# learningmatter-mit/surface-sampling

Hardware: AMD Instinct MI355X
Metric: MC energy-evaluations/sec (SrTiO3(001) ~250-atom slabs, 3-model PaiNN ensemble E+F incl. neighbor list) (higher is better)
Workload: dtype f32 via fp16x2-split MFMA (3 products), fp32 accumulate; neighbor decisions f64; 1 GPU; SrTiO3(001) PaiNN x3, 256 batched independent chains per GPU (BASELINE configs[3]), 248-272 atoms/chain; chains_per_gpu=256, atoms_per_gpu=66503, edges_per_gpu=2747786, slots_per_gpu=2836316, models=3, streams_per_gpu=2, parallelism=one GPU, no collective

## Files before the change

### surface-sampling_amd/csrc/api_batch.hip

```cpp
#include <cmath>
#include <cstdio>

#include "cell_dev.h"
#include "ewald_dev.h"

using namespace vssr;

extern "C" {

int vssr_batch_upload(vssr_handle *h, int32_t n_cfg, const int32_t *n_atoms, const int32_t *Z, const double *pos,
                      const double *cell, const uint8_t *pbc) {
    if (int rc = check_kind(h, KINDS_EVAL, __func__)) return rc;
    if (n_cfg < 1 || !n_atoms || !Z || !pos || !cell || !pbc) return set_err(h, VSSR_E_BADARG, "null or empty batch");
    VSSR_HIP(h, hipSetDevice(h->device));
    VSSR_HIP(h, hipStreamSynchronize(h->stream));
    h->batch_valid = false;
    h->ran = false;
    h->md_vel_valid = false;
    std::vector<int> start(n_cfg + 1, 0);
    for (int b = 0; b < n_cfg; ++b) {
        if (n_atoms[b] < 1) return set_err(h, VSSR_E_BADARG, "configuration %d has %d atoms", b, n_atoms[b]);
        if ((int64_t)start[b] + n_atoms[b] > 2000000000LL) return set_err(h, VSSR_E_BADARG, "batch too large");
        start[b + 1] = start[b] + n_atoms[b];
    }
// ... 573 lines not shown
        if (l == 0 && h->l0_used)
            return set_err(h, VSSR_E_STATE, "phi0 is not materialised (layer-0 species factorisation is active)");
        src = sv.phi[l]; per_atom = F3;
    }
    else if ((l = layer_of("s_msg")) >= 0) { src = sv.s_msg[l]; per_atom = F; }
    else if ((l = layer_of("v_msg")) >= 0) { src = sv.v_msg[l]; per_atom = F3; }
    else if ((l = layer_of("s_upd")) >= 0) { src = sv.s_in[l + 1]; per_atom = F; }
    else if ((l = layer_of("v_upd")) >= 0) {
        if (l == h->num_conv - 1 && !h->debug_keep)
            return set_err(h, VSSR_E_STATE, "v_upd of the last block is not materialised (nothing consumes it; create the handle with VSSR_DEBUG_KEEP=1)");
        src = sv.v_in[l + 1]; per_atom = F3;
    }
    else if (nm == "e_atom") { src = sv.e_atom; per_atom = 1; }
    else if (nm == "sbar_msg0") { src = sv.sbar_msg_l0; per_atom = F; }
    else if (nm == "vbar_msg0") { src = sv.vbar_msg; per_atom = F3; }
    else return set_err(h, VSSR_E_BADARG, "unknown intermediate '%s'", name);
    size_t n = N * per_atom;
    *n_out = (int64_t)n;
    if (!dst) return VSSR_OK;
    if ((int64_t)n > cap) return set_err(h, VSSR_E_BADARG, "buffer too small for '%s'", name);
    VSSR_HIP(h, hipMemcpy(dst, src + (size_t)model * n, n * sizeof(float), hipMemcpyDeviceToHost));
    return VSSR_OK;
}

}
```

### surface-sampling_amd/csrc/api_painn.hip

```cpp
#include <cmath>

#include "vssr_internal.h"

namespace vssr {

static void transpose(const float *src, int rows, int cols, float *dst) {
    for (int r = 0; r < rows; ++r)
        for (int c = 0; c < cols; ++c) dst[(size_t)c * rows + r] = src[(size_t)r * cols + c];
}

static int upload_weights(vssr_handle *h, const vssr_painn_config *cfg) {
    const int M = cfg->n_models, L = cfg->num_conv, R = cfg->n_rbf, H = cfg->readout_hidden, NE = cfg->n_embed;
    const size_t per_layer = (size_t)F * F + F + (size_t)F3 * F + F3 + (size_t)F3 * R + F3 + 2 * (size_t)F * F +
                             (size_t)F * 2 * F + F + (size_t)F3 * F + F3;
    const size_t blob_len = (size_t)NE * F + L * per_layer + (size_t)H * F + H + H + 1;
    if (cfg->weights_len != blob_len)
        return set_err(h, VSSR_E_BADARG, "weights_len %llu does not match the layout (%zu floats)",
                       (unsigned long long)cfg->weights_len, blob_len);
    const size_t t_per_layer = (size_t)F * F + (size_t)F * F3 + 2 * (size_t)F * F + (size_t)2 * F * F + (size_t)F * F3;
    const size_t img_len = blob_len + L * t_per_layer + (size_t)F * H;
    std::vector<float> img(img_len * M);
    std::vector<ModelW> table(M);
    if (h->weights.ensure(img.size() * sizeof(float)))
        return set_err(h, VSSR_E_NOMEM, "weights: out of device memory");
// ... 123 lines not shown
}

static void read_env_knobs(vssr_handle *h) {
    if (const char *e = getenv("VSSR_PAINN_PATH")) h->painn_general = h->painn_general || strcmp(e, "general") == 0;
    if (const char *e = getenv("VSSR_EDGE_IMPL")) h->edge_impl = (strcmp(e, "gather") == 0) ? 0 : 1;
    if (const char *e = getenv("VSSR_L0_FACTORISE")) h->l0_enabled = atoi(e);
    if (h->painn_general) h->l0_enabled = 0;
    if (const char *e = getenv("VSSR_UPD_SAVE")) h->upd_save = atoi(e);
    if (const char *e = getenv("VSSR_DEBUG_KEEP")) h->debug_keep = atoi(e);
    if (const char *e = getenv("VSSR_EDGE_FS16_MAX")) h->fs16_max_atoms = atoi(e);
    if (const char *e = getenv("VSSR_EDGE_FS8_MAX")) h->fs8_max_atoms = atoi(e);
    if (const char *e = getenv("VSSR_EDGE_BWD_MPASS")) h->bwd_multi_pass = atoi(e);
    if (const char *e = getenv("VSSR_EDGE_SUB_CHUNK")) { const int c = atoi(e); if (c >= 8) { h->sub_chunk_fwd = c; h->sub_chunk_bwd = c; } }
    if (const char *e = getenv("VSSR_EDGE_FWD_2PASS")) { const int w = atoi(e); h->fwd_two_pass = (w == 8 || w == 16) ? w : w ? 16 : 0; }
    if (const char *e = getenv("VSSR_EDGE_FWD_GRID")) h->edge_fwd_grid = max(atoi(e), 0);
}

}

using namespace vssr;

extern "C" {

int vssr_create(const vssr_painn_config *cfg, vssr_handle **out) {
    if (!cfg || !out) return set_err(nullptr, VSSR_E_BADARG, "null argument");
    *out = nullptr;
    if (cfg->struct_size != sizeof(vssr_painn_config))
        return set_err(nullptr, VSSR_E_BADARG, "vssr_painn_config size mismatch (%u vs %zu)", cfg->struct_size,
                       sizeof(vssr_painn_config));
    if (cfg->feat_dim < 16 || cfg->feat_dim > 256 || cfg->feat_dim % 16 != 0 || cfg->n_rbf < 1 || cfg->n_rbf > 32)
// ... 39 lines not shown
```

### surface-sampling_amd/csrc/mfma16.h

```cpp
#ifndef VSSR_MFMA16_H
#define VSSR_MFMA16_H
#include "vssr_internal.h"

namespace vssr {

typedef float f32x4 __attribute__((ext_vector_type(4)));
typedef float f32x2 __attribute__((ext_vector_type(2)));
typedef unsigned u32x4 __attribute__((ext_vector_type(4)));
typedef unsigned u32x2 __attribute__((ext_vector_type(2)));
typedef _Float16 f16x8 __attribute__((ext_vector_type(8)));
typedef _Float16 f16x2 __attribute__((ext_vector_type(2)));

constexpr int TA = 32;
constexpr int NW = 8;
constexpr int NTHREADS = 64 * NW;
constexpr int PADH = 8;

#ifndef VSSR_FAST_SIGMOID
#define VSSR_FAST_SIGMOID 1
#endif
__device__ __forceinline__ float sigm(float x) {
#if VSSR_FAST_SIGMOID && defined(__HIP_DEVICE_COMPILE__)
    constexpr float C_HI = -1.44269502162933349609375f;
    constexpr float C_LO = -1.9259629911266175e-08f;
// ... 120 lines not shown
    }
}
template <int NROWS, class Sat>
__device__ __forceinline__ void rows_store_split(const Planes &P, int col0, const float4 (&v)[NROWS * (F / 4) / NTHREADS],
                                                 Sat &sat) {
    constexpr int NIT = NROWS * (F / 4) / NTHREADS;
#pragma unroll
    for (int it = 0; it < NIT; ++it) {
        const int idx = threadIdx.x + it * NTHREADS;
        store_split4<SAT_COOP>(P, idx >> 5, col0 + 4 * (idx & 31), v[it], sat);
    }
}

constexpr int FT = F + 4;
template <int NROWS, class Fn>
__device__ __forceinline__ void stage_rows(const float *T, Fn fn) {
    constexpr int NIT = NROWS * (F / 4) / NTHREADS;
    static_assert(NROWS * (F / 4) % NTHREADS == 0, "tile pass must divide evenly");
#pragma unroll
    for (int it = 0; it < NIT; ++it) {
        const int idx = threadIdx.x + it * NTHREADS, row = idx >> 5, c4 = idx & 31;
        fn(row, 4 * c4, *reinterpret_cast<const float4 *>(T + row * FT + 4 * c4));
    }
}

template <int NROWS, class Ld, class St>
__device__ __forceinline__ void stage_rows_residual(const float *T, Ld ld, St st) {
    constexpr int NIT = NROWS * (F / 4) / NTHREADS;
    static_assert(NROWS * (F / 4) % NTHREADS == 0, "tile pass must divide evenly");
    float4 r[NIT];
#pragma unroll
    for (int it = 0; it < NIT; ++it) {
        const int idx = threadIdx.x + it * NTHREADS;
        r[it] = ld(idx >> 5, 4 * (idx & 31));
    }
#pragma unroll
    for (int it = 0; it < NIT; ++it) {
        const int idx = threadIdx.x + it * NTHREADS, row = idx >> 5, c4 = idx & 31;
        st(row, 4 * c4, *reinterpret_cast<const float4 *>(T + row * FT + 4 * c4), r[it]);
// ... 38 lines not shown
```

### surface-sampling_amd/csrc/painn.hip

```cpp
#include "vssr_internal.h"

namespace vssr {

constexpr int T = NODE_TILE;
constexpr int RB = 21;
constexpr int ECHUNK = 16;
constexpr float PI_F = 3.14159265358979323846f;

__device__ inline float sigmoidf_(float x) { return 1.f / (1.f + expf(-x)); }
__device__ inline float swishf_(float x) { return x * sigmoidf_(x); }
__device__ inline float dswishf_(float x) {
    float sg = sigmoidf_(x);
    return sg * fmaf(x, 1.f - sg, 1.f);
}

__global__ void __launch_bounds__(128) k_embed(int N, const int *__restrict__ Z, const ModelW *__restrict__ MW,
                                               float *__restrict__ s0, float *__restrict__ v0) {
    int i = blockIdx.x, m = blockIdx.y, f = threadIdx.x;
    const ModelW &W = MW[m];
    size_t a = (size_t)m * N + i;
    s0[a * F + f] = W.embed[(size_t)Z[i] * F + f];
    v0[(a * 3 + 0) * F + f] = 0.f;
    v0[(a * 3 + 1) * F + f] = 0.f;
    v0[(a * 3 + 2) * F + f] = 0.f;
// ... 612 lines not shown
    const float *e_excl = h->excl_vol ? sv.e_excl : (const float *)nullptr;
    if (!(fused && want_forces)) {
        P.begin(KC_READOUT, st);
        if (fused) launch_readout_mfma(st, N, M, av, MW, sv.s_in[L], e_excl, sv.e_atom);
        else
            hipLaunchKernelGGL(k_readout, g_tile, blk, 0, st, N, H, av, MW, sv.s_in[L], sv.e_excl, h->excl_vol, sv.e_atom,
                               sv.sbar);
        P.end(st);
    }

    if (want_forces) {
        float *sb_buf[2] = {sv.sbar_msg, sv.sbar};
        for (int l = L - 1; l >= 0; --l) {
            float *sbar_msg_l = fused ? sb_buf[(L - 1 - l) & 1] : sv.sbar_msg;
            const float *sbar_msg_up = sb_buf[(L - l) & 1];
            P.begin(KC_UPDATE_BWD, st);
            if (!fused)
                launch_update_bwd_mfma(st, N, M, l, 0, (int)(l == L - 1), av, MW, sv.s_msg[l], sv.v_msg[l], sv.sbar, sv.vbar,
                                       nullptr, nullptr, nullptr, nullptr, sbar_msg_l, sv.vbar_msg, nullptr, nullptr);
            else if (l == L - 1 && fuse_last)
                launch_update_bwd_mfma(st, N, M, l, 3, 1, av, MW, sv.s_msg[l], sv.v_msg[l], nullptr, sv.vbar, nullptr, nullptr,
                                       e_excl, sv.e_atom, sbar_msg_l, sv.vbar_msg, sv.s_in[L], nullptr);
            else if (l == L - 1)
                launch_update_bwd_mfma(st, N, M, l, 1, 1, av, MW, sv.s_msg[l], sv.v_msg[l], nullptr, sv.vbar, sv.s_in[L], nullptr,
                                       e_excl, sv.e_atom, sbar_msg_l, sv.vbar_msg, nullptr, save_of(l));
            else
                launch_update_bwd_mfma(st, N, M, l, 2, 0, av, MW, sv.s_msg[l], sv.v_msg[l], sbar_msg_up, sv.vbar, sv.s_in[l + 1],
                                       sv.phibar, nullptr, nullptr, sbar_msg_l, sv.vbar_msg, nullptr, save_of(l));
            P.end(st);
            sv.sbar_msg_l0 = sbar_msg_l;
            P.begin((l == 0 && l0_fact) ? KC_L0_BWD : KC_EDGE_BWD, st);
            int accumulate = (l != L - 1);
            if (l == 0 && l0_fact) {
                rc = l0_run_reverse(h, G, (int)(L == 1), (int)partial, sbar_msg_l, sv.vbar_msg, sv.gbar);
                if (rc) return rc;
            } else if (l == 0)
                hipLaunchKernelGGL(k_edge_bwd<true>, g_atom, blk, 0, st, N, l, accumulate, MW, G, counters,
                                   h->cutoff, h->excl_vol, h->excl_sigma, h->excl_power, sv.v_in[l], sv.phi[l],
                                   sbar_msg_l, sv.vbar_msg, sv.phibar, sv.vbar, sv.gbar,
                                   (long long)h->slot_cap, -1, (int)partial);
            else {
                for (int cls = 0; cls < EDGE_MFMA_BCLASSES; ++cls)
                    launch_edge_bwd_mfma(st, cls, N, bcls_list[cls], h->n_bclass[cls], M, l, h->max_bclass_atoms[cls], MW, G, counters,
                                         (int)(h->slot_cap - 1), sv.v_in[l], sv.phi[l], sbar_msg_l, sv.vbar_msg, sv.phibar, sv.vbar,
                                         h->d_gpart.as<float>(), (long long)h->slot_cap, n_groups, (L - 1 - l) * per_set,
                                         cls == EDGE_BCLASS_FS16P ? h->d_bundle_subb.as<int4>() : (const int4 *)nullptr,
                                         h->sub_chunk_bwd ? h->sub_chunk_bwd : sub_chunk_max_bwd());
                if (n_gather)
                    hipLaunchKernelGGL(k_edge_bwd<false>, g_atom, blk, 0, st, N, l, accumulate, MW, G, counters,
// ... 49 lines not shown
```

### surface-sampling_amd/csrc/painn_l0.hip

```cpp
#include "mfma16.h"

namespace vssr {

constexpr int KP = 24;
constexpr int TBLK = 4 * KP;

template <int NZ>
__global__ void __launch_bounds__(96)
k_l0_accum(GraphView G, const int *__restrict__ counters, float *__restrict__ T) {
    constexpr int nz = NZ;
    if (counters[2] || !G.act.atom(blockIdx.x)) return;
    const int i = blockIdx.x, comp = threadIdx.x / KP, kap = threadIdx.x % KP;
    float acc[NZ];
#pragma unroll
    for (int z = 0; z < NZ; ++z) acc[z] = 0.f;
    auto erec_c = [&](int idx) -> float4 {
#if defined(__HIP_DEVICE_COMPILE__)
        typedef const f32x4 __attribute__((address_space(4))) *cp;
        const f32x4 v = reinterpret_cast<cp>(reinterpret_cast<uintptr_t>(G.erec))[idx];
        return make_float4(v.x, v.y, v.z, v.w);
#else
        return G.erec[idx];
#endif
    };
// ... 17 lines not shown
            r[u] = G.rho[(size_t)(e + u) * KP + kap];
            zi[u] = (zw >> (8 * u)) & 255;
        }
#pragma unroll
        for (int u = 0; u < 4; ++u) {
            const float uu = comp == 0 ? 1.f : comp == 1 ? er[u].x : comp == 2 ? er[u].y : er[u].z;
            const float val = r[u] * uu;
#pragma unroll
            for (int z = 0; z < NZ; ++z) acc[z] += (z == zi[u]) ? val : 0.f;
        }
    }
#pragma unroll
    for (int z = 0; z < NZ; ++z) T[((size_t)i * nz + z) * TBLK + comp * KP + kap] = acc[z];
}

constexpr int L0_TILE_U4 = 1024;

__global__ void __launch_bounds__(NTHREADS)
k_l0_fwd16(int N, int M, int nz, ActiveView av, const int *__restrict__ counters, const int *__restrict__ Z,
           const int *__restrict__ zlist, const ModelW *__restrict__ MW, const uint4 *__restrict__ A16, int n_embed,
           const float *__restrict__ T, float *__restrict__ s_msg, float *__restrict__ v_msg) {
    extern __shared__ __attribute__((aligned(16))) _Float16 ldsh[];
    if (counters[2]) return;
    const int K = 32 * nz, a0 = blockIdx.x * TA;
    if (!av.tile(min(a0, N - 1), min(a0 + TA - 1, N - 1))) return;
    const Planes Ts = make_planes(ldsh, TA, K), Tv = make_planes(ldsh + plane_halves(TA, K), 3 * TA, K);
    const LaneGeo L;
    SatTrack sat;
    const int lane = threadIdx.x & 63, r = lane & 15, g = lane >> 4;
    for (int t = threadIdx.x; t < TA * nz * 4 * 8; t += NTHREADS) {
        const int k4 = t & 7, comp = (t >> 3) & 3, z = (t >> 5) % nz, a = t / (32 * nz);
        float4 val = make_float4(0.f, 0.f, 0.f, 0.f);
// ... 271 lines not shown
            case 3: hipLaunchKernelGGL(k_l0_accum<3>, dim3(N), dim3(96), 0, st, G, cnt, T); break;
            case 4: hipLaunchKernelGGL(k_l0_accum<4>, dim3(N), dim3(96), 0, st, G, cnt, T); break;
            case 5: hipLaunchKernelGGL(k_l0_accum<5>, dim3(N), dim3(96), 0, st, G, cnt, T); break;
            case 6: hipLaunchKernelGGL(k_l0_accum<6>, dim3(N), dim3(96), 0, st, G, cnt, T); break;
            case 7: hipLaunchKernelGGL(k_l0_accum<7>, dim3(N), dim3(96), 0, st, G, cnt, T); break;
            default: hipLaunchKernelGGL(k_l0_accum<L0_MAX_SPECIES>, dim3(N), dim3(96), 0, st, G, cnt, T); break;
        }
    }
    const size_t lds_fwd = sizeof(_Float16) * (plane_halves(TA, 32 * nz) + plane_halves(3 * TA, 32 * nz));
    hipLaunchKernelGGL(k_l0_fwd16, dim3((N + TA - 1) / TA), dim3(NTHREADS), lds_fwd, st, N, M, nz, G.act, h->d_counters.as<int>(),
                       h->d_Z.as<int>(), h->d_zlist.as<int>(), h->model_table.as<ModelW>(), h->d_l0A.as<uint4>(), h->n_embed,
                       h->d_l0T.as<float>(), s_msg, v_msg);
    return VSSR_OK;
}

int l0_run_reverse(vssr_handle *h, const GraphView &G, int first_write, int fresh_mfma, const float *sbar_msg, const float *vbar_msg,
                   float4 *gbar) {
    const int N = h->n_atoms, M = h->n_models, nz = h->l0_nz;
    hipStream_t st = h->stream;
    const size_t lds_q = sizeof(_Float16) * (plane_halves(TA, F) + plane_halves(3 * TA, F));
    hipLaunchKernelGGL(k_l0_q16, dim3((N + TA - 1) / TA, M), dim3(NTHREADS), lds_q, st, N, nz, G.act, h->d_counters.as<int>(),
                       h->d_zlist.as<int>(), h->d_l0At.as<uint4>(), h->n_embed, sbar_msg, vbar_msg, h->d_l0Q.as<float>());
    if (sizeof(float) * 4 * M * nz * TBLK > 48 * 1024)
        VSSR_HIP(h, hipFuncSetAttribute((const void *)k_l0_bwd, hipFuncAttributeMaxDynamicSharedMemorySize, 160 * 1024));
    hipLaunchKernelGGL(k_l0_bwd, dim3((N + 3) / 4), dim3(256), sizeof(float) * 4 * M * nz * TBLK, st, N, M, nz, first_write, fresh_mfma,
                       h->excl_vol, h->cutoff, G, h->d_counters.as<int>(), h->d_l0Q.as<float>(), gbar, (long long)h->slot_cap);
    return VSSR_OK;
}

}
```

### surface-sampling_amd/csrc/painn_node_mfma.hip

```cpp
#include "mfma16.h"

#ifdef PHASE_TIMING
__device__ unsigned long long g_phase[64];
#define PH_INIT unsigned long long ph_t = wall_clock64();
#define PH_RESET ph_t = wall_clock64();
#define PH(k) { const unsigned long long ph_n = wall_clock64(); if (threadIdx.x == 0) atomicAdd(&g_phase[k], ph_n - ph_t); ph_t = wall_clock64(); }
extern "C" int vssr_debug_phases(unsigned long long *out, int reset) {
    if (hipMemcpyFromSymbol(out, HIP_SYMBOL(g_phase), sizeof(unsigned long long) * 64) != hipSuccess) return -1;
    if (reset) { unsigned long long z[64] = {}; if (hipMemcpyToSymbol(HIP_SYMBOL(g_phase), z, sizeof(z)) != hipSuccess) return -1; }
    return 0;
}
#else
#define PH_INIT
#define PH_RESET
#define PH(k)
#endif

namespace vssr {

template <int NRT, int NCT>
struct GemmShape {
    static constexpr int NT = NRT * NCT, NACC = NT >= 3 ? 1 : 2;
};
template <int NRT, int NCT, int NPRE>
// ... 691 lines not shown
    extern __shared__ __attribute__((aligned(16))) _Float16 ldsh[];
    const int m = blockIdx.y, a0 = blockIdx.x * TA;
    if (!av.tile(min(a0, N - 1), min(a0 + TA - 1, N - 1))) return;
    const LaneGeo L;
    SatTrack sat;
    const size_t mN = (size_t)m * N;
    const Planes xs = make_planes(ldsh, TA, F), hp = make_planes(ldsh + plane_halves(TA, F), TA, RH);
    float *red = reinterpret_cast<float *>(ldsh + plane_halves(TA, F) + plane_halves(TA, RH));
    load_rows_split<TA>(xs, 0, [&](int row) { return s + (mN + min(a0 + row, N - 1)) * F; }, sat);
    __syncthreads();
    f32x4 sb[2];
    readout_head<2, false>(MW[m], xs, hp, red, L, a0, N, mN, e_excl, e_atom, sb, sat);
    sat.commit(av, a0, N);
}

template <int MODE, int RT, bool SAVED = false>
__global__ void __launch_bounds__(NTHREADS) __attribute__((amdgpu_waves_per_eu(RT == 1 ? 4 : 2, RT == 1 ? 4 : 2)))
k_update_bwd_mfma(int N, int l, int vbar_is_zero, ActiveView av, const ModelW *__restrict__ MW, const float *__restrict__ s_msg,
                  const float *__restrict__ v_msg, const float *__restrict__ sbar_src, const float *__restrict__ vbar,
                  const float *__restrict__ s_next, const float *__restrict__ phibar, const float *__restrict__ e_excl,
                  float *__restrict__ e_atom, float *__restrict__ sbar_msg, float *__restrict__ vbar_msg,
                  float *__restrict__ s_last, const f32x4 *__restrict__ save) {
    static_assert(!SAVED || RT == 2, "the saved layout is that of the 32-atom forward kernel");
    constexpr bool FUSED = MODE == 3;
    static_assert(!FUSED || (!SAVED && RT == 2), "the fused last block runs its own forward pass on 32-atom tiles");
    static_assert(MODE != 1 || SAVED, "without stored intermediates the last layer is MODE 3");
    extern __shared__ __attribute__((aligned(16))) _Float16 ldsh[];
    constexpr int TA = 16 * RT, OFF_VT = UpdLds<RT>::OFF_VT, OFF_AS = UpdLds<RT>::OFF_AS, UPD_LDS_HALVES = UpdLds<RT>::HALVES;
    const int m = blockIdx.y, a0 = blockIdx.x * TA;
    if (!av.tile(min(a0, N - 1), min(a0 + TA - 1, N - 1))) return;
    const LaneGeo L;
    constexpr int BPF = MODE == 0 ? 0 : UPD_PF;
    SatNone unwatched;
    const LayerW &W = MW[m].layer[l];
    const size_t mN = (size_t)m * N;
    PH_INIT
    f32x4 sb[RT];
    if (MODE != 1 && !FUSED) {
// ... 235 lines not shown
            store_split4(ab, x * TA + row, L.col0, ub, sat);
            store_split4(ab, x * TA + row, F + L.col0, vb2, sat);
        }
    }
    sat.commit(av, a0, N);
    PH(29)
    __syncthreads();
    PH(30)
    f32x4 out[3 * RT][1];
    zero_acc(out);
    {
        const uint4 *wp[1] = {WTILE(UVt, L.w, 2 * F)};
        gemm16<2 * F, 3 * RT, 1, BPF>(ab, wp, out);
    }
    PH(31)
    __syncthreads();
    PH(32)
    float *T = reinterpret_cast<float *>(ldsh);
#pragma unroll
    for (int t = 0; t < RT; ++t) {
        const int row = L.row(t);
        *reinterpret_cast<f32x4 *>(T + row * FT + L.col0) = sb[t] + hbar[t][0];
#pragma unroll
        for (int x = 0; x < 3; ++x) *reinterpret_cast<f32x4 *>(T + (TA * (1 + x) + row) * FT + L.col0) = out[RT * x + t][0];
    }
    __syncthreads();
    stage_rows<4 * TA>(T, [&](int row, int col, const float4 &d) {
        const int q = row / TA, a = a0 + row % TA;
        if (a >= N) return;
        if (q == 0) {
            *reinterpret_cast<float4 *>(sbar_msg + (mN + a) * F + col) = d;
        } else {
            const size_t off = ((mN + a) * 3 + (q - 1)) * F + col;
            float4 r = make_float4(0.f, 0.f, 0.f, 0.f);
            if (!vbar_is_zero) r = *reinterpret_cast<const float4 *>(VB + (row - TA) * FT + col);
            *reinterpret_cast<float4 *>(vbar_msg + off) = make_float4(r.x + d.x, r.y + d.y, r.z + d.z, r.w + d.w);
        }
    });
    PH(33)
}

void pack_mfma_tiles16(const float *Wsrc, int rows, int K, unsigned *dst) {
    auto split2 = [](float x, unsigned (&p)[2]) {
        const _Float16 h = (_Float16)x;
        const _Float16 l = (_Float16)(x - (float)h);
        unsigned short hb, lb;
        memcpy(&hb, &h, 2);
        memcpy(&lb, &l, 2);
        p[0] = hb; p[1] = lb;
    };
    const int ntile = rows / 16, nq = K / 32;
    for (int tile = 0; tile < ntile; ++tile)
        for (int q = 0; q < nq; ++q)
            for (int lane = 0; lane < 64; ++lane)
// ... 31 lines not shown
    VSSR_HIP(h, hipFuncSetAttribute((const void *)k_update_fwd_mfma<0>, hipFuncAttributeMaxDynamicSharedMemorySize,
                                    (int)node_mfma_lds_bytes(6)));
    VSSR_HIP(h, hipFuncSetAttribute((const void *)k_update_fwd_mfma<1>, hipFuncAttributeMaxDynamicSharedMemorySize,
                                    (int)node_mfma_lds_bytes(6)));
    VSSR_HIP(h, hipFuncSetAttribute((const void *)k_update_fwd_mfma<2>, hipFuncAttributeMaxDynamicSharedMemorySize,
                                    (int)node_mfma_lds_bytes(6)));
#define SET_UPD(MODE)                                                                                                     \
    VSSR_HIP(h, hipFuncSetAttribute((const void *)k_update_bwd_mfma<MODE, 2>, hipFuncAttributeMaxDynamicSharedMemorySize, \
                                    (int)node_mfma_lds_bytes(3)));
    SET_UPD(0) SET_UPD(2) SET_UPD(3)
#undef SET_UPD
    VSSR_HIP(h, hipFuncSetAttribute((const void *)k_update_bwd_mfma<1, 2, true>, hipFuncAttributeMaxDynamicSharedMemorySize,
                                    (int)node_mfma_lds_bytes(3)));
    VSSR_HIP(h, hipFuncSetAttribute((const void *)k_update_bwd_mfma<2, 2, true>, hipFuncAttributeMaxDynamicSharedMemorySize,
                                    (int)node_mfma_lds_bytes(3)));
    VSSR_HIP(h, hipFuncSetAttribute((const void *)k_readout_mfma, hipFuncAttributeMaxDynamicSharedMemorySize,
                                    (int)node_mfma_lds_bytes(4)));
    return VSSR_OK;
}

void launch_msg_mlp_mfma(hipStream_t st, int N, int M, int l, const ActiveView &av, const ModelW *MW, const float *s_in,
                         float *phi) {
    hipLaunchKernelGGL((k_msg_mlp_mfma<2, 0>), dim3((N + TA - 1) / TA, M), dim3(NTHREADS), node_mfma_lds_bytes(0), st, N, l, av, MW,
                       s_in, phi);
}
void launch_msg_mlp_bwd_mfma(hipStream_t st, int N, int M, int l, const ActiveView &av, const ModelW *MW, const float *s_in,
                             const float *phibar, const float *sbar_msg, float *sbar_in) {
    hipLaunchKernelGGL(k_msg_mlp_bwd_mfma, dim3((N + TA - 1) / TA, M), dim3(NTHREADS), node_mfma_lds_bytes(1), st, N, l, av, MW,
                       s_in, phibar, sbar_msg, sbar_in);
}
// ... 6 lines not shown
    else if (!v_out && !sv)
        hipLaunchKernelGGL(k_update_fwd_mfma<2>, dim3((N + TA - 1) / TA, M), dim3(NTHREADS), node_mfma_lds_bytes(6), st, N, l,
                           av, MW, s_msg, v_msg, s_out, v_out, phi_next, sv);
    else
        hipLaunchKernelGGL(k_update_fwd_mfma<0>, dim3((N + TA - 1) / TA, M), dim3(NTHREADS), node_mfma_lds_bytes(6), st, N, l,
                           av, MW, s_msg, v_msg, s_out, v_out, phi_next, sv);
}
void launch_readout_mfma(hipStream_t st, int N, int M, const ActiveView &av, const ModelW *MW, const float *s,
                         const float *e_excl, float *e_atom) {
    hipLaunchKernelGGL(k_readout_mfma, dim3((N + TA - 1) / TA, M), dim3(NTHREADS), node_mfma_lds_bytes(4), st, N, av, MW, s,
                       e_excl, e_atom);
}
void launch_update_bwd_mfma(hipStream_t st, int N, int M, int l, int mode, int vbar_is_zero, const ActiveView &av, const ModelW *MW,
                            const float *s_msg, const float *v_msg, const float *sbar_src, const float *vbar,
                            const float *s_next, const float *phibar, const float *e_excl, float *e_atom,
                            float *sbar_msg, float *vbar_msg, float *s_last, const void *save) {
    const f32x4 *sv = reinterpret_cast<const f32x4 *>(save);
    if (mode == 1 || mode == 3) vbar_is_zero = 1;
#if defined(UPD_BWD_RT) && UPD_BWD_RT == 1
    if (!sv && mode == 2) {
        const dim3 grid1((N + 15) / 16, M), blk1(NTHREADS);
        const size_t lds1 = sizeof(_Float16) * UpdLds<1>::HALVES + sizeof(float) * 3 * 16 * FT;
        static bool once = [] {
            (void)hipFuncSetAttribute((const void *)k_update_bwd_mfma<2, 1, false>, hipFuncAttributeMaxDynamicSharedMemorySize, 80 * 1024);
            return true;
        }();
        (void)once;
        hipLaunchKernelGGL((k_update_bwd_mfma<2, 1, false>), grid1, blk1, lds1, st, N, l, vbar_is_zero, av, MW, s_msg, v_msg, sbar_src,
                           vbar, s_next, phibar, e_excl, e_atom, sbar_msg, vbar_msg, s_last, sv);
        return;
    }
#endif
    const dim3 grid((N + TA - 1) / TA, M), blk(NTHREADS);
    const size_t lds = node_mfma_lds_bytes(3);
#define LAUNCH_UPD(MODE, SAVED)                                                                                             \
    hipLaunchKernelGGL((k_update_bwd_mfma<MODE, 2, SAVED>), grid, blk, lds, st, N, l, vbar_is_zero, av, MW, s_msg, v_msg, sbar_src, \
                       vbar, s_next, phibar, e_excl, e_atom, sbar_msg, vbar_msg, s_last, sv)
    if (mode == 1) LAUNCH_UPD(1, true);
    else if (mode == 2) { if (sv) LAUNCH_UPD(2, true); else LAUNCH_UPD(2, false); }
    else if (mode == 3) LAUNCH_UPD(3, false);
    else LAUNCH_UPD(0, false);
#undef LAUNCH_UPD
}

}
```

### surface-sampling_amd/csrc/vssr_internal.h

```cpp
#pragma once

#include <hip/hip_runtime.h>

#include <cstdint>
#include <cstdio>
#include <cstdlib>
#include <cstring>
#include <initializer_list>
#include <memory>
#include <string>
#include <type_traits>
#include <utility>
#include <vector>

#include "../../include/vssr_eval.h"

namespace vssr {

constexpr int F = 128;
constexpr int F3 = 3 * F;
constexpr int MAX_LAYERS = 4;
constexpr int MAX_MODELS = 8;
constexpr int RB_MAX = 24;
constexpr int NODE_TILE = 8;
constexpr int L0_MAX_SPECIES = 8;

struct LayerW {
    const float *W1, *W1t, *b1;
    const float *W2, *W2t, *b2;
    const float *Wd, *bd;
    const float *U, *Ut, *V, *Vt;
    const float *W3, *W3t, *b3;
    const float *W4, *W4t, *b4;
    const uint4 *qW1, *qW2, *qU, *qV, *qW3, *qW4, *qW1t, *qW2t, *qW4t, *qW3t, *qUVt;
    const uint4 *wd16;
};
struct ModelW {
    const float *embed;
    LayerW layer[MAX_LAYERS];
    const float *W5, *W5t, *b5, *w6, *b6;
// ... 290 lines not shown

    bool batch_valid = false, ran = false;
    int n_cfg = 0, n_atoms = 0;
    std::vector<int> h_n_atoms, h_cfg_start;
    vssr::DevBuf d_pos, d_wpos, d_wrap, d_Z, d_atom_cfg, d_cfg_start, d_cell, d_invcell, d_nimg, d_pbc;
    vssr::DevBuf d_deg, d_row_start, d_edge, d_edge_S, d_rev, d_counters, d_tile_sums;
    vssr::DevBuf d_erec, d_rho, d_dist, d_rho16, d_drho16, d_zslot, d_bundle, d_excl;
    vssr::DevBuf d_bundle_sub;
    int bwd_multi_pass = 1;
    int sub_chunk_fwd = 0, sub_chunk_bwd = 0;
    vssr::DevBuf d_bundle_subb;
    int fwd_two_pass = 16;
    int edge_fwd_grid = -1;
    vssr::DevBuf d_hits;
    int l0_enabled = 1, l0_nz = 0;
    bool l0_used = false;
    vssr::DevBuf d_l0A, d_l0At;
    vssr::DevBuf d_zmap, d_zlist;
    vssr::DevBuf d_l0T, d_l0Q;
    vssr::DevBuf d_opt_state, d_opt_vec, d_bfgs_q, d_bfgs_b, d_fixed, d_relax_steps, d_relax_conv, d_active;
    const unsigned char *active_mask = nullptr;
    int relax_regrows = 0;
    long long relax_lockstep = 0;
    int relax_compactions = 0;
    vssr::DevBuf d_cmp;
    vssr::DevBuf d_cm;
    long long relax_chain_evals = 0;
    int traj_interval = 0, traj_records = 0, traj_B = 0, traj_N = 0;
    vssr::DevBuf d_traj_pos, d_traj_f, d_traj_e, d_traj_n;
    bool graph_partial = false;
// ... 140 lines not shown
}
template <class P>
using force_type = std::remove_cv_t<std::remove_pointer_t<P>>;
void eam_build_spline(const double *f, int n, double delta, double *spl );
int relax_fire(vssr_handle *h, const vssr_fire_params &p, const uint8_t *fixed_host, uint32_t want);
int relax_bfgs(vssr_handle *h, const vssr_bfgs_params &p, const uint8_t *fixed_host, uint32_t want);
int driver_guard(vssr_handle *h, const char *func);
int driver_open(vssr_handle *h, const uint8_t *fixed_host, int steps_ints_per_chain, const uint8_t *&fixed, uint32_t want);
int driver_close(vssr_handle *h, bool partial);
int relax_regrow(vssr_handle *h, int cap, long long &it, int window);
int relax_results(vssr_handle *h, bool partial, double *pos_out, std::initializer_list<int32_t *> cols);
int relax_cg(vssr_handle *h, const vssr_cg_params *cp, const uint8_t *fixed_host, uint32_t want);
int relax_bfgsls(vssr_handle *h, const vssr_bfgsls_params *bp, const uint8_t *fixed_host, uint32_t want);
bool chain_min_supported(const vssr_handle *h);
int chain_min_cg(vssr_handle *h, const vssr_cg_params *cp, const uint8_t *fixed_host, uint32_t want);
int node_mfma_init(vssr_handle *h);
void launch_msg_mlp_mfma(hipStream_t st, int N, int M, int l, const ActiveView &av, const ModelW *MW, const float *s_in,
                         float *phi);
void launch_msg_mlp_bwd_mfma(hipStream_t st, int N, int M, int l, const ActiveView &av, const ModelW *MW, const float *s_in,
                             const float *phibar, const float *sbar_msg, float *sbar_in);
void launch_update_fwd_mfma(hipStream_t st, int N, int M, int l, const ActiveView &av, const ModelW *MW, const float *s_msg,
                            const float *v_msg, float *s_out, float *v_out, float *phi_next, void *save);
size_t update_save_bytes(int N, int M);
bool readout_mfma_supported(int hidden);
void launch_readout_mfma(hipStream_t st, int N, int M, const ActiveView &av, const ModelW *MW, const float *s, const float *e_excl,
                         float *e_atom);
void launch_update_bwd_mfma(hipStream_t st, int N, int M, int l, int mode, int vbar_is_zero, const ActiveView &av, const ModelW *MW,
                            const float *s_msg, const float *v_msg, const float *sbar_src, const float *vbar,
                            const float *s_next, const float *phibar, const float *e_excl, float *e_atom,
                            float *sbar_msg, float *vbar_msg, float *s_last, const void *save);
void pack_mfma_tiles16(const float *Wsrc, int rows, int K, unsigned *dst );
void build_wd16(const float *Wd, const float *bd, unsigned *dst );
void l0_build_tables(const float *blob_embed, const float *W1, const float *b1, const float *W2, const float *b2,
                     const float *Wd, const float *bd, int n_embed, float *A, float *At);
void l0_pack_tables(const float *A, int n_embed, unsigned *A16, unsigned *At16);
size_t l0_packed_dwords(int n_embed);
int l0_mfma_init(vssr_handle *h);
int l0_run_forward(vssr_handle *h, const GraphView &G, float *s_msg, float *v_msg);
int l0_run_reverse(vssr_handle *h, const GraphView &G, int first_write, int fresh_mfma, const float *sbar_msg, const float *vbar_msg,
                   float4 *gbar);
int edge_mfma_init(vssr_handle *h);
enum { EDGE_CLASS_FS16 = 0, EDGE_CLASS_FS16M = 1, EDGE_CLASS_FS8 = 2, EDGE_CLASS_FS4 = 3, EDGE_CLASS_GATHER = 4, EDGE_CLASSES = 5,
       EDGE_MFMA_CLASSES = 4 };
enum { EDGE_BCLASS_FS16 = 0, EDGE_BCLASS_FS8 = 1, EDGE_BCLASS_FS4 = 2, EDGE_BCLASS_FS16P = 3, EDGE_BCLASS_GATHER = 4, EDGE_BCLASSES = 5,
       EDGE_MFMA_BCLASSES = 4 };
__host__ __device__ constexpr int edge_bclass_slices(int c) { return (c == EDGE_BCLASS_FS16 || c == EDGE_BCLASS_FS16P) ? 8 : c == EDGE_BCLASS_FS8 ? 16 : c == EDGE_BCLASS_FS4 ? 32 : 1; }
int edge_bclass_of(int n_atoms);
int edge_class_of(int n_atoms);
constexpr int SUB_MAX_PASSES = 4;
__host__ __device__ constexpr int sub_chunk_max(int width) { return width == 16 ? 400 : 784; }
__host__ __device__ constexpr int sub_chunk_max_bwd() { return 550; }
__host__ __device__ constexpr int sub_passes(int n_atoms, int chunk_max) { return (n_atoms + chunk_max - 1) / chunk_max; }
__host__ __device__ constexpr int sub_chunk(int n_atoms, int chunk_max) { return (n_atoms + sub_passes(n_atoms, chunk_max) - 1) / sub_passes(n_atoms, chunk_max); }
int edge_class_groups(int cls);
void launch_edge_bwd_mfma(hipStream_t st, int cls, int N, const int *list, int n_list, int M, int l, int max_atoms,
// ... 11 lines not shown
```

Before: 25850 evaluations/s.

## Fuse layer-0 species Q projection into the mode-2 update backward kernel tail

When layer-0 species factorisation is active, the layer-0 update-backward kernel now also computes the Q tensor. It keeps its sbar/vbar output tile in LDS as fp16 split planes and runs an MFMA tail against the At16 species tables, so the separate k_l0_q16 launch is skipped. This removes one kernel launch and the global round trip that re-read sbar_msg and vbar_msg. In exchange the update kernel grows longer, uses more registers, and reuses its LDS for the tail. The new path can be turned off with the VSSR_L0_Q_FUSED environment variable, and an l0_q debug readout is added.

```diff
diff --git a/surface-sampling_amd/csrc/api_batch.hip b/surface-sampling_amd/csrc/api_batch.hip
--- a/surface-sampling_amd/csrc/api_batch.hip
+++ b/surface-sampling_amd/csrc/api_batch.hip
@@ -611,6 +611,11 @@
     else if (nm == "e_atom") { src = sv.e_atom; per_atom = 1; }
     else if (nm == "sbar_msg0") { src = sv.sbar_msg_l0; per_atom = F; }
     else if (nm == "vbar_msg0") { src = sv.vbar_msg; per_atom = F3; }
+    else if (nm == "l0_q") {
+        if (!h->l0_used || !h->d_l0Q.p)
+            return set_err(h, VSSR_E_STATE, "l0_q is not materialised (layer-0 species factorisation is not active)");
+        src = h->d_l0Q.as<float>(); per_atom = (size_t)h->l0_nz * TBLK;
+    }
     else return set_err(h, VSSR_E_BADARG, "unknown intermediate '%s'", name);
     size_t n = N * per_atom;
     *n_out = (int64_t)n;
diff --git a/surface-sampling_amd/csrc/api_painn.hip b/surface-sampling_amd/csrc/api_painn.hip
--- a/surface-sampling_amd/csrc/api_painn.hip
+++ b/surface-sampling_amd/csrc/api_painn.hip
@@ -161,6 +161,7 @@
     if (const char *e = getenv("VSSR_EDGE_SUB_CHUNK")) { const int c = atoi(e); if (c >= 8) { h->sub_chunk_fwd = c; h->sub_chunk_bwd = c; } }
     if (const char *e = getenv("VSSR_EDGE_FWD_2PASS")) { const int w = atoi(e); h->fwd_two_pass = (w == 8 || w == 16) ? w : w ? 16 : 0; }
     if (const char *e = getenv("VSSR_EDGE_FWD_GRID")) h->edge_fwd_grid = max(atoi(e), 0);
+    if (const char *e = getenv("VSSR_L0_Q_FUSED")) h->l0_q_fused = atoi(e);
 }
 
 }
diff --git a/surface-sampling_amd/csrc/mfma16.h b/surface-sampling_amd/csrc/mfma16.h
--- a/surface-sampling_amd/csrc/mfma16.h
+++ b/surface-sampling_amd/csrc/mfma16.h
@@ -158,15 +158,17 @@
 
 constexpr int FT = F + 4;
 template <int NROWS, class Fn>
-__device__ __forceinline__ void stage_rows(const float *T, Fn fn) {
+__device__ __forceinline__ void stage_rows(const float *T, Fn fn, int tid) {
     constexpr int NIT = NROWS * (F / 4) / NTHREADS;
     static_assert(NROWS * (F / 4) % NTHREADS == 0, "tile pass must divide evenly");
 #pragma unroll
     for (int it = 0; it < NIT; ++it) {
-        const int idx = threadIdx.x + it * NTHREADS, row = idx >> 5, c4 = idx & 31;
+        const int idx = tid + it * NTHREADS, row = idx >> 5, c4 = idx & 31;
         fn(row, 4 * c4, *reinterpret_cast<const float4 *>(T + row * FT + 4 * c4));
     }
 }
+template <int NROWS, class Fn>
+__device__ __forceinline__ void stage_rows(const float *T, Fn fn) { stage_rows<NROWS>(T, fn, threadIdx.x); }
 
 template <int NROWS, class Ld, class St>
 __device__ __forceinline__ void stage_rows_residual(const float *T, Ld ld, St st) {
diff --git a/surface-sampling_amd/csrc/painn.hip b/surface-sampling_amd/csrc/painn.hip
--- a/surface-sampling_amd/csrc/painn.hip
+++ b/surface-sampling_amd/csrc/painn.hip
@@ -650,6 +650,8 @@
         for (int l = L - 1; l >= 0; --l) {
             float *sbar_msg_l = fused ? sb_buf[(L - 1 - l) & 1] : sv.sbar_msg;
             const float *sbar_msg_up = sb_buf[(L - l) & 1];
+            const bool l0q = l == 0 && l0_fact && fused && l < L - 1 && !keep && h->l0_q_fused && update_bwd_has_l0q_tail();
+            const L0QTail q0 = l0q ? l0_q_tail_args(h) : L0QTail();
             P.begin(KC_UPDATE_BWD, st);
             if (!fused)
                 launch_update_bwd_mfma(st, N, M, l, 0, (int)(l == L - 1), av, MW, sv.s_msg[l], sv.v_msg[l], sv.sbar, sv.vbar,
@@ -662,13 +664,13 @@
                                        e_excl, sv.e_atom, sbar_msg_l, sv.vbar_msg, nullptr, save_of(l));
             else
                 launch_update_bwd_mfma(st, N, M, l, 2, 0, av, MW, sv.s_msg[l], sv.v_msg[l], sbar_msg_up, sv.vbar, sv.s_in[l + 1],
-                                       sv.phibar, nullptr, nullptr, sbar_msg_l, sv.vbar_msg, nullptr, save_of(l));
+                                       sv.phibar, nullptr, nullptr, sbar_msg_l, sv.vbar_msg, nullptr, save_of(l), l0q ? &q0 : nullptr);
             P.end(st);
             sv.sbar_msg_l0 = sbar_msg_l;
             P.begin((l == 0 && l0_fact) ? KC_L0_BWD : KC_EDGE_BWD, st);
             int accumulate = (l != L - 1);
             if (l == 0 && l0_fact) {
-                rc = l0_run_reverse(h, G, (int)(L == 1), (int)partial, sbar_msg_l, sv.vbar_msg, sv.gbar);
+                rc = l0_run_reverse(h, G, (int)(L == 1), (int)partial, sbar_msg_l, sv.vbar_msg, sv.gbar, l0q);
                 if (rc) return rc;
             } else if (l == 0)
                 hipLaunchKernelGGL(k_edge_bwd<true>, g_atom, blk, 0, st, N, l, accumulate, MW, G, counters,
diff --git a/surface-sampling_amd/csrc/painn_l0.hip b/surface-sampling_amd/csrc/painn_l0.hip
--- a/surface-sampling_amd/csrc/painn_l0.hip
+++ b/surface-sampling_amd/csrc/painn_l0.hip
@@ -1,9 +1,6 @@
 #include "mfma16.h"
 
 namespace vssr {
-
-constexpr int KP = 24;
-constexpr int TBLK = 4 * KP;
 
 template <int NZ>
 __global__ void __launch_bounds__(96)
@@ -55,8 +52,6 @@
     for (int z = 0; z < NZ; ++z) T[((size_t)i * nz + z) * TBLK + comp * KP + kap] = acc[z];
 }
 
-constexpr int L0_TILE_U4 = 1024;
-
 __global__ void __launch_bounds__(NTHREADS)
 k_l0_fwd16(int N, int M, int nz, ActiveView av, const int *__restrict__ counters, const int *__restrict__ Z,
            const int *__restrict__ zlist, const ModelW *__restrict__ MW, const uint4 *__restrict__ A16, int n_embed,
@@ -358,13 +353,25 @@
     return VSSR_OK;
 }
 
+L0QTail l0_q_tail_args(vssr_handle *h) {
+    L0QTail q;
+    q.At16 = h->d_l0At.as<uint4>();
+    q.zlist = h->d_zlist.as<int>();
+    q.nz = h->l0_nz;
+    q.n_embed = h->n_embed;
+    q.Q = h->d_l0Q.as<float>();
+    return q;
+}
+
 int l0_run_reverse(vssr_handle *h, const GraphView &G, int first_write, int fresh_mfma, const float *sbar_msg, const float *vbar_msg,
-                   float4 *gbar) {
+                   float4 *gbar, bool q_done) {
     const int N = h->n_atoms, M = h->n_models, nz = h->l0_nz;
     hipStream_t st = h->stream;
-    const size_t lds_q = sizeof(_Float16) * (plane_halves(TA, F) + plane_halves(3 * TA, F));
-    hipLaunchKernelGGL(k_l0_q16, dim3((N + TA - 1) / TA, M), dim3(NTHREADS), lds_q, st, N, nz, G.act, h->d_counters.as<int>(),
-                       h->d_zlist.as<int>(), h->d_l0At.as<uint4>(), h->n_embed, sbar_msg, vbar_msg, h->d_l0Q.as<float>());
+    if (!q_done) {
+        const size_t lds_q = sizeof(_Float16) * (plane_halves(TA, F) + plane_halves(3 * TA, F));
+        hipLaunchKernelGGL(k_l0_q16, dim3((N + TA - 1) / TA, M), dim3(NTHREADS), lds_q, st, N, nz, G.act, h->d_counters.as<int>(),
+                           h->d_zlist.as<int>(), h->d_l0At.as<uint4>(), h->n_embed, sbar_msg, vbar_msg, h->d_l0Q.as<float>());
+    }
     if (sizeof(float) * 4 * M * nz * TBLK > 48 * 1024)
         VSSR_HIP(h, hipFuncSetAttribute((const void *)k_l0_bwd, hipFuncAttributeMaxDynamicSharedMemorySize, 160 * 1024));
     hipLaunchKernelGGL(k_l0_bwd, dim3((N + 3) / 4), dim3(256), sizeof(float) * 4 * M * nz * TBLK, st, N, M, nz, first_write, fresh_mfma,
diff --git a/surface-sampling_amd/csrc/painn_node_mfma.hip b/surface-sampling_amd/csrc/painn_node_mfma.hip
--- a/surface-sampling_amd/csrc/painn_node_mfma.hip
+++ b/surface-sampling_amd/csrc/painn_node_mfma.hip
@@ -729,14 +729,20 @@
     sat.commit(av, a0, N);
 }
 
-template <int MODE, int RT, bool SAVED = false>
+constexpr int L0Q_OFF_X = 4 * TA * FT * (int)(sizeof(float) / sizeof(_Float16));
+constexpr int L0Q_SPECIES = 3;
+static_assert(sizeof(_Float16) * (L0Q_OFF_X + plane_halves(TA, F) + plane_halves(3 * TA, F)) <=
+                  sizeof(_Float16) * UpdLds<2>::HALVES + sizeof(float) * 3 * TA * FT,
+              "output tile + X planes of the Q tail fit the kernel's LDS (planes + fp32 vbar tile)");
+template <int MODE, int RT, bool SAVED = false, bool L0Q = false>
 __global__ void __launch_bounds__(NTHREADS) __attribute__((amdgpu_waves_per_eu(RT == 1 ? 4 : 2, RT == 1 ? 4 : 2)))
 k_update_bwd_mfma(int N, int l, int vbar_is_zero, ActiveView av, const ModelW *__restrict__ MW, const float *__restrict__ s_msg,
                   const float *__restrict__ v_msg, const float *__restrict__ sbar_src, const float *__restrict__ vbar,
                   const float *__restrict__ s_next, const float *__restrict__ phibar, const float *__restrict__ e_excl,
                   float *__restrict__ e_atom, float *__restrict__ sbar_msg, float *__restrict__ vbar_msg,
-                  float *__restrict__ s_last, const f32x4 *__restrict__ save) {
+                  float *__restrict__ s_last, const f32x4 *__restrict__ save, L0QTail q0) {
     static_assert(!SAVED || RT == 2, "the saved layout is that of the 32-atom forward kernel");
+    static_assert(!L0Q || (MODE == 2 && RT == 2 && !SAVED), "the Q tail exists for the recomputing mode-2 kernel on 32-atom tiles");
     constexpr bool FUSED = MODE == 3;
     static_assert(!FUSED || (!SAVED && RT == 2), "the fused last block runs its own forward pass on 32-atom tiles");
     static_assert(MODE != 1 || SAVED, "without stored intermediates the last layer is MODE 3");
@@ -1002,17 +1008,60 @@
         gemm16<2 * F, 3 * RT, 1, BPF>(ab, wp, out);
     }
     PH(31)
+    if constexpr (L0Q) {
+#pragma unroll
+        for (int t = 0; t < RT; ++t)
+#pragma unroll
+            for (int x = 0; x < 3; ++x) {
+                f32x4 vbo = {0.f, 0.f, 0.f, 0.f};
+                if (!vbar_is_zero) vbo = *reinterpret_cast<const f32x4 *>(VB + (x * TA + L.row(t)) * FT + L.col0);
+                out[RT * x + t][0] += vbo;
+            }
+    }
     __syncthreads();
     PH(32)
     float *T = reinterpret_cast<float *>(ldsh);
-#pragma unroll
-    for (int t = 0; t < RT; ++t) {
-        const int row = L.row(t);
-        *reinterpret_cast<f32x4 *>(T + row * FT + L.col0) = sb[t] + hbar[t][0];
-#pragma unroll
-        for (int x = 0; x < 3; ++x) *reinterpret_cast<f32x4 *>(T + (TA * (1 + x) + row) * FT + L.col0) = out[RT * x + t][0];
-    }
-    __syncthreads();
+    const Planes Xs = make_planes(ldsh + L0Q_OFF_X, TA, F), Xv = make_planes(ldsh + L0Q_OFF_X + plane_halves(TA, F), 3 * TA, F);
+    {
+        SatTrack satq;
+#pragma unroll
+        for (int t = 0; t < RT; ++t) {
+            const int row = L.row(t);
+            const f32x4 so = sb[t] + hbar[t][0];
+            *reinterpret_cast<f32x4 *>(T + row * FT + L.col0) = so;
+            if constexpr (L0Q) store_split4(Xs, row, L.col0, so, satq);
+#pragma unroll
+            for (int x = 0; x < 3; ++x) {
+                *reinterpret_cast<f32x4 *>(T + (TA * (1 + x) + row) * FT + L.col0) = out[RT * x + t][0];
+                if constexpr (L0Q) store_split4(Xv, x * TA + row, L.col0, out[RT * x + t][0], satq);
+            }
+        }
+        if constexpr (L0Q) satq.commit(av, a0, N);
+    }
+    __syncthreads();
+    constexpr int QCT = 2 * L0Q_SPECIES;
+    int qtid = threadIdx.x;
+    if constexpr (L0Q) asm volatile("" : "+v"(qtid));
+    const int qw = __builtin_amdgcn_readfirstlane(qtid >> 6), qlane = qtid & 63;
+    const uint4 *qwb[QCT];
+    u32x4 qbb[2][QCT][2];
+    auto q_tiles = [&](int z0) {
+#pragma unroll
+        for (int j = 0; j < QCT; ++j)
+            qwb[j] = q0.At16 + (((size_t)m * q0.n_embed + q0.zlist[min(z0 + (j >> 1), q0.nz - 1)]) * 2 + (qw < 2 ? 0 : 1)) * L0_TILE_U4 +
+                     (size_t)(j & 1) * 512 + qlane;
+    };
+    auto q_load = [&](int buf, int c) {
+#pragma unroll
+        for (int j = 0; j < QCT; ++j)
+#pragma unroll
+            for (int pc = 0; pc < 2; ++pc) qbb[buf][j][pc] = gload4u(qwb[j] + (c * 2 + pc) * 64);
+    };
+    if constexpr (L0Q) {
+        q_tiles(0);
+        q_load(0, 0);
+        __builtin_amdgcn_sched_barrier(0);
+    }
     stage_rows<4 * TA>(T, [&](int row, int col, const float4 &d) {
         const int q = row / TA, a = a0 + row % TA;
         if (a >= N) return;
@@ -1020,12 +1069,60 @@
             *reinterpret_cast<float4 *>(sbar_msg + (mN + a) * F + col) = d;
         } else {
             const size_t off = ((mN + a) * 3 + (q - 1)) * F + col;
-            float4 r = make_float4(0.f, 0.f, 0.f, 0.f);
-            if (!vbar_is_zero) r = *reinterpret_cast<const float4 *>(VB + (row - TA) * FT + col);
-            *reinterpret_cast<float4 *>(vbar_msg + off) = make_float4(r.x + d.x, r.y + d.y, r.z + d.z, r.w + d.w);
-        }
-    });
+            if constexpr (L0Q) {
+                *reinterpret_cast<float4 *>(vbar_msg + off) = d;
+            } else {
+                float4 r = make_float4(0.f, 0.f, 0.f, 0.f);
+                if (!vbar_is_zero) r = *reinterpret_cast<const float4 *>(VB + (row - TA) * FT + col);
+                *reinterpret_cast<float4 *>(vbar_msg + off) = make_float4(r.x + d.x, r.y + d.y, r.z + d.z, r.w + d.w);
+            }
+        }
+    }, qtid);
     PH(33)
+    if constexpr (L0Q) {
+        const int r = qlane & 15, g = qlane >> 4;
+        const Planes &P = qw < 2 ? Xs : Xv;
+        const int prow = (qw < 2 ? 16 * qw : 16 * (qw - 2)) + r;
+        const _Float16 *xh = P.h + prow * P.ld + 8 * g, *xl = P.l + prow * P.ld + 8 * g;
+        const int comp = qw < 2 ? 0 : 1 + ((qw - 2) >> 1), tt = qw < 2 ? qw : (qw - 2) & 1;
+#pragma unroll 1
+        for (int z0 = 0; z0 < q0.nz; z0 += L0Q_SPECIES) {
+            if (z0) {
+                q_tiles(z0);
+                q_load(0, 0);
+            }
+            f32x4 acc[QCT];
+#pragma unroll
+            for (int j = 0; j < QCT; ++j) acc[j] = (f32x4){0.f, 0.f, 0.f, 0.f};
+#pragma unroll
+            for (int c = 0; c < F / 32; ++c) {
+                if (c + 1 < F / 32) q_load((c + 1) & 1, c + 1);
+                const u32x4 ah = *reinterpret_cast<const u32x4 *>(xh + 32 * c), al = *reinterpret_cast<const u32x4 *>(xl + 32 * c);
+                __builtin_amdgcn_sched_barrier(0);
+#pragma unroll
+                for (int k = 0; k < 3; ++k)
+#pragma unroll
+                    for (int j = 0; j < QCT; ++j) {
+                        acc[j] = mfma16(k == 1 ? al : ah, qbb[c & 1][j][k == 0 ? 1 : 0], acc[j]);
+                        __builtin_amdgcn_sched_barrier(0);
+                    }
+                asm volatile("; gemm16_group_end");
+                __builtin_amdgcn_sched_barrier(0);
+            }
+#pragma unroll
+            for (int j = 0; j < QCT; ++j) {
+                const int z = z0 + (j >> 1), kap = 16 * (j & 1) + r;
+                if (z < q0.nz && kap < KP) {
+#pragma unroll
+                    for (int i = 0; i < 4; ++i) {
+                        const int a_ = a0 + 16 * tt + 4 * g + i;
+                        if (a_ < N) q0.Q[((((size_t)m * N + a_) * q0.nz + z) * 4 + comp) * KP + kap] = acc[j][i];
+                    }
+                }
+            }
+        }
+        PH(34)
+    }
 }
 
 void pack_mfma_tiles16(const float *Wsrc, int rows, int K, unsigned *dst) {
@@ -1087,6 +1184,8 @@
                                     (int)node_mfma_lds_bytes(3)));
     VSSR_HIP(h, hipFuncSetAttribute((const void *)k_update_bwd_mfma<2, 2, true>, hipFuncAttributeMaxDynamicSharedMemorySize,
                                     (int)node_mfma_lds_bytes(3)));
+    VSSR_HIP(h, hipFuncSetAttribute((const void *)k_update_bwd_mfma<2, 2, false, true>, hipFuncAttributeMaxDynamicSharedMemorySize,
+                                    (int)node_mfma_lds_bytes(3)));
     VSSR_HIP(h, hipFuncSetAttribute((const void *)k_readout_mfma, hipFuncAttributeMaxDynamicSharedMemorySize,
                                     (int)node_mfma_lds_bytes(4)));
     return VSSR_OK;
@@ -1123,8 +1222,9 @@
 void launch_update_bwd_mfma(hipStream_t st, int N, int M, int l, int mode, int vbar_is_zero, const ActiveView &av, const ModelW *MW,
                             const float *s_msg, const float *v_msg, const float *sbar_src, const float *vbar,
                             const float *s_next, const float *phibar, const float *e_excl, float *e_atom,
-                            float *sbar_msg, float *vbar_msg, float *s_last, const void *save) {
+                            float *sbar_msg, float *vbar_msg, float *s_last, const void *save, const L0QTail *q0) {
     const f32x4 *sv = reinterpret_cast<const f32x4 *>(save);
+    const L0QTail qt = q0 ? *q0 : L0QTail();
     if (mode == 1 || mode == 3) vbar_is_zero = 1;
 #if defined(UPD_BWD_RT) && UPD_BWD_RT == 1
     if (!sv && mode == 2) {
@@ -1136,20 +1236,28 @@
         }();
         (void)once;
         hipLaunchKernelGGL((k_update_bwd_mfma<2, 1, false>), grid1, blk1, lds1, st, N, l, vbar_is_zero, av, MW, s_msg, v_msg, sbar_src,
-                           vbar, s_next, phibar, e_excl, e_atom, sbar_msg, vbar_msg, s_last, sv);
+                           vbar, s_next, phibar, e_excl, e_atom, sbar_msg, vbar_msg, s_last, sv, qt);
         return;
     }
 #endif
     const dim3 grid((N + TA - 1) / TA, M), blk(NTHREADS);
     const size_t lds = node_mfma_lds_bytes(3);
-#define LAUNCH_UPD(MODE, SAVED)                                                                                             \
-    hipLaunchKernelGGL((k_update_bwd_mfma<MODE, 2, SAVED>), grid, blk, lds, st, N, l, vbar_is_zero, av, MW, s_msg, v_msg, sbar_src, \
-                       vbar, s_next, phibar, e_excl, e_atom, sbar_msg, vbar_msg, s_last, sv)
-    if (mode == 1) LAUNCH_UPD(1, true);
-    else if (mode == 2) { if (sv) LAUNCH_UPD(2, true); else LAUNCH_UPD(2, false); }
-    else if (mode == 3) LAUNCH_UPD(3, false);
-    else LAUNCH_UPD(0, false);
+#define LAUNCH_UPD(MODE, SAVED, L0Q)                                                                                        \
+    hipLaunchKernelGGL((k_update_bwd_mfma<MODE, 2, SAVED, L0Q>), grid, blk, lds, st, N, l, vbar_is_zero, av, MW, s_msg, v_msg, sbar_src, \
+                       vbar, s_next, phibar, e_excl, e_atom, sbar_msg, vbar_msg, s_last, sv, qt)
+    if (mode == 1) LAUNCH_UPD(1, true, false);
+    else if (mode == 2) { if (sv) LAUNCH_UPD(2, true, false); else if (q0) LAUNCH_UPD(2, false, true); else LAUNCH_UPD(2, false, false); }
+    else if (mode == 3) LAUNCH_UPD(3, false, false);
+    else LAUNCH_UPD(0, false, false);
 #undef LAUNCH_UPD
 }
 
-}
+bool update_bwd_has_l0q_tail() {
+#if defined(UPD_BWD_RT) && UPD_BWD_RT == 1
+    return false;
+#else
+    return true;
+#endif
+}
+
+}
diff --git a/surface-sampling_amd/csrc/vssr_internal.h b/surface-sampling_amd/csrc/vssr_internal.h
--- a/surface-sampling_amd/csrc/vssr_internal.h
+++ b/surface-sampling_amd/csrc/vssr_internal.h
@@ -24,6 +24,9 @@
 constexpr int RB_MAX = 24;
 constexpr int NODE_TILE = 8;
 constexpr int L0_MAX_SPECIES = 8;
+constexpr int KP = 24;
+constexpr int TBLK = 4 * KP;
+constexpr int L0_TILE_U4 = 1024;
 
 struct LayerW {
     const float *W1, *W1t, *b1;
@@ -344,6 +347,7 @@
     int edge_fwd_grid = -1;
     vssr::DevBuf d_hits;
     int l0_enabled = 1, l0_nz = 0;
+    int l0_q_fused = 1;
     bool l0_used = false;
     vssr::DevBuf d_l0A, d_l0At;
     vssr::DevBuf d_zmap, d_zlist;
@@ -514,6 +518,12 @@
 int relax_bfgsls(vssr_handle *h, const vssr_bfgsls_params *bp, const uint8_t *fixed_host, uint32_t want);
 bool chain_min_supported(const vssr_handle *h);
 int chain_min_cg(vssr_handle *h, const vssr_cg_params *cp, const uint8_t *fixed_host, uint32_t want);
+struct L0QTail {
+    const uint4 *At16 = nullptr;
+    const int *zlist = nullptr;
+    int nz = 0, n_embed = 0;
+    float *Q = nullptr;
+};
 int node_mfma_init(vssr_handle *h);
 void launch_msg_mlp_mfma(hipStream_t st, int N, int M, int l, const ActiveView &av, const ModelW *MW, const float *s_in,
                          float *phi);
@@ -528,7 +538,8 @@
 void launch_update_bwd_mfma(hipStream_t st, int N, int M, int l, int mode, int vbar_is_zero, const ActiveView &av, const ModelW *MW,
                             const float *s_msg, const float *v_msg, const float *sbar_src, const float *vbar,
                             const float *s_next, const float *phibar, const float *e_excl, float *e_atom,
-                            float *sbar_msg, float *vbar_msg, float *s_last, const void *save);
+                            float *sbar_msg, float *vbar_msg, float *s_last, const void *save, const L0QTail *q0 = nullptr);
+bool update_bwd_has_l0q_tail();
 void pack_mfma_tiles16(const float *Wsrc, int rows, int K, unsigned *dst );
 void build_wd16(const float *Wd, const float *bd, unsigned *dst );
 void l0_build_tables(const float *blob_embed, const float *W1, const float *b1, const float *W2, const float *b2,
@@ -538,7 +549,8 @@
 int l0_mfma_init(vssr_handle *h);
 int l0_run_forward(vssr_handle *h, const GraphView &G, float *s_msg, float *v_msg);
 int l0_run_reverse(vssr_handle *h, const GraphView &G, int first_write, int fresh_mfma, const float *sbar_msg, const float *vbar_msg,
-                   float4 *gbar);
+                   float4 *gbar, bool q_done);
+L0QTail l0_q_tail_args(vssr_handle *h);
 int edge_mfma_init(vssr_handle *h);
 enum { EDGE_CLASS_FS16 = 0, EDGE_CLASS_FS16M = 1, EDGE_CLASS_FS8 = 2, EDGE_CLASS_FS4 = 3, EDGE_CLASS_GATHER = 4, EDGE_CLASSES = 5,
        EDGE_MFMA_CLASSES = 4 };
```

After: 25680 evaluations/s. No clear change (-0.6%).
